# kubernetes-sigs/kube-batch

Measured on AMD Instinct MI355X. Metric: pod-node scoring evals/sec + binds/sec, 100k tasks x 10k nodes snapshot, higher is better.
Workload: dtype f64+i64

## Files before the change

### kube-batch_amd/csrc/kb_commit_sel.hip

```cpp
#include <string.h>

#include <algorithm>

#include "kb_k9.hpp"
#include "kb_repair.hpp"

#define K9S_PREP0 5u
#define K9S_PREPS 3u
#define K9S_SPIN_LIMIT (1u << 21)

__device__ __forceinline__ uint32_t k9s_ld(const uint32_t *p) { return __hip_atomic_load(p, __ATOMIC_ACQUIRE, __HIP_MEMORY_SCOPE_WORKGROUP); }
__device__ __forceinline__ void k9s_st(uint32_t *p, uint32_t v) { __hip_atomic_store(p, v, __ATOMIC_RELEASE, __HIP_MEMORY_SCOPE_WORKGROUP); }
__device__ __forceinline__ bool k9s_wait(K9Sync &Y, const uint32_t *p, uint32_t need, uint32_t nap = 1u) {
  uint32_t spins = 0;
  for (;;) {
    if (k9s_ld(p) >= need) return true;
    if ((++spins & 31u) == 0u) {
      if (k9s_ld(&Y.stop) | k9s_ld(&Y.err)) return k9s_ld(p) >= need;
      if (spins > K9S_SPIN_LIMIT) { k9s_st(&Y.err, 1u); return false; }
    }
    if (nap == 0u) { } else if (nap == 1u) __builtin_amdgcn_s_sleep(1); else if (nap <= 4u) __builtin_amdgcn_s_sleep(4); else __builtin_amdgcn_s_sleep(16);
  }
}

__global__ void __launch_bounds__(K9_THREADS) k_commit_select(const K9KernArgs ka) {
  KbCommitArgs a = ka.hot;
  {
    const unsigned char __attribute__((address_space(4))) *kp = (const unsigned char __attribute__((address_space(4))) *)__builtin_amdgcn_kernarg_segment_ptr();
    a.dev = (const KbDev *)(kp + offsetof(K9KernArgs, dev));
    a.round = (const KbRound *)(kp + offsetof(K9KernArgs, round));
  }
  extern __shared__ __align__(16) unsigned char k9_smem[];
  if ((blockIdx.x & 7u) != 0u && a.round->lists_ready != nullptr) {
    const uint32_t row = blockIdx.x - 1u - blockIdx.x / 8u;
    if (row < a.n_mrows && !KB_CHAIN_BROKEN(*a.round)) kb_repair_row<K9_THREADS>(*a.dev, *a.round, k9_smem, row, threadIdx.x);
    return;
  }
  if (k9_preamble(a)) return;
  const uint32_t tid = threadIdx.x, lane = tid & 63, wave = tid >> 6;
  const uint32_t S = a.n_mrows, W = a.n_rows;
  const K9Layout lo = k9_layout(W, S, a.L, a.NP, a.R, true);
  unsigned char *k9_base_ = k9_smem;
  K9_LDS_VIEWS(lo)
  (void)shp; (void)S; (void)dk; (void)ckey; (void)cpos;
  K9Sel &X = *reinterpret_cast<K9Sel *>(k9_smem + lo.sel);
  K9Sync &Y = X.sync;
  const unsigned long long t_start = wall_clock64();
#ifdef KB_K9_TRACE
  unsigned long long t_stage[2] = {0ull, 0ull};
  const bool staged = k9_prologue(a, lo, k9_smem, tid, 0u, t_stage);
#else
  const bool staged = k9_prologue(a, lo, k9_smem, tid, 0u);
#endif
// ... 18 lines not shown
    if (brk) atomicOr(&X.brk[tid >> 5], 1u << (tid & 31));
  }
  __syncthreads();
  if (tid < W) {
    uint32_t w = tid >> 5, mword = X.brk[w] & (0xFFFFFFFFu >> (31u - (tid & 31u)));
    while (mword == 0u) { w--; mword = X.brk[w]; }
    const uint32_t p = 32u * w + (31u - (uint32_t)__clz((int)mword));
    if ((tid - p) % K9_SEL_MAXRUN == 0u) atomicOr(&X.stm[tid >> 5], 1u << (tid & 31));
  }
  __syncthreads();
  if (tid < W && ((X.stm[tid >> 5] >> (tid & 31)) & 1u)) {
    uint32_t kidx = (uint32_t)__popc(X.stm[tid >> 5] & ((1u << (tid & 31)) - 1u));
    for (uint32_t w = 0; w < (tid >> 5); w++) kidx += (uint32_t)__popc(X.stm[w]);
    X.runs[kidx] = (uint16_t)tid;
  }
  __syncthreads();
  uint32_t K = 0;
  for (uint32_t w = 0; w < 8; w++) K += (uint32_t)__popc(X.stm[w]);
  {
    uint4 rr = make_uint4(0u, 0u, 0u, 0u);
    uint32_t i0c = 0u;
    uint32_t rlen = 0u;
    if (tid < K) { i0c = X.runs[tid]; rr = rinfo[i0c]; rlen = ((tid + 1u < K) ? (uint32_t)X.runs[tid + 1u] : W) - i0c; }
    __syncthreads();
    if (tid < K) rinfo[tid] = make_uint4(i0c | (rlen << 16), rr.y, rr.z, rr.w);
    __syncthreads();
  }

#ifdef KB_K9_TRACE
  uint32_t tacc[10] = {0, 0, 0, 0, 0, 0, 0, 0, 0, 0};
  const unsigned long long t_tab = wall_clock64();
  tacc[1] = (uint32_t)(t_stage[0] - t_start); tacc[9] = (uint32_t)(t_stage[1] - t_stage[0]); tacc[2] = (uint32_t)(t_tab - t_stage[1]);
  unsigned long long tlast = __builtin_readcyclecounter();
#define K9S_TR(k, t0) do { if (lane == 0) atomicAdd(&X.tr[k], (uint32_t)(__builtin_readcyclecounter() - (t0))); } while (0)
#define K9S_NOW() __builtin_readcyclecounter()
#else
#define K9S_TR(k, t0) do { (void)(t0); } while (0)
#define K9S_NOW() 0ull
#endif
#ifndef KB_K9_NAP_PREP
#define KB_K9_NAP_PREP 1u
#endif
  constexpr uint32_t nap_prep = KB_K9_NAP_PREP, nap_dk = 1u;
#if !defined(KB_K9_PRIO) || KB_K9_PRIO
#define K9S_SETPRIO(p) __builtin_amdgcn_s_setprio(p)
#else
#define K9S_SETPRIO(p) do { } while (0)
#endif
  const unsigned long long lt = (1ull << lane) - 1ull;
  gptrd gi, gr;
  { const KbDev &d = *a.dev; gi = (gptrd)d.idle; gr = (gptrd)d.rel; }
#define K9S_RUN_HEADER_OF(ri_)                                                                                         \
  const uint32_t hx_ = (uint32_t)__builtin_amdgcn_readfirstlane((int)(ri_).x);                                          \
  const uint32_t i0 = hx_ & 0xFFFFu, r = hx_ >> 16, s = (uint32_t)__builtin_amdgcn_readfirstlane((int)(ri_).y);          \
  const uint32_t fl0 = (uint32_t)__builtin_amdgcn_readfirstlane((int)(ri_).z), km0 = (uint32_t)__builtin_amdgcn_readfirstlane((int)(ri_).w); \
  const bool plain0 = (fl0 & 1u) && (km0 == 0u || (fl0 & 4u));                                                         \
  const bool sel_run = !a.backfill && plain0 && r >= 2u && a.whole;             \
  (void)sel_run; (void)i0;
#define K9S_RUN_SHAPE(kk)                                                                                              \
  const K9Shape sh = shapes[s];                                                                                        \
  const double *si = sinit + (size_t)s * RS;                                                                           \
  const double *rres = rowres + ((kk) % K9S_PREPS) * (uint32_t)a.R;    \
  const double *rqv = plain0 ? si : rres + 2;                                             \
  (void)rqv; (void)rres;
#define K9S_RUN_HEADER(kk)                                                                                             \
  const uint4 ri_ = rinfo[(kk)];                                                                                       \
  K9S_RUN_HEADER_OF(ri_)                                                                                               \
  K9S_RUN_SHAPE(kk)

  if (wave == 0) {
    K9S_SETPRIO(3);
    uint32_t nd = 0, n_dirty_rows = 0, n_runs = 0, n_slow = 0, i_end = 0, reason_end = KB_REASON_DONE;
    uint32_t prev_nd0 = 0, prev_pc = 0;
    bool prev_chg = true;
    bool prev_all = false;
    uint4 hd_next = rinfo[0];
    for (uint32_t k = 0; k < K; k++) {
      uint32_t lane_i = tid;
      asm volatile("" : "+v"(lane_i));
      const uint4 hd = hd_next;
      if (k + 1u < K) hd_next = rinfo[k + 1u];
      K9S_RUN_HEADER_OF(hd)
      K9_STAMP(3);
      {
        uint32_t spins = 0;
        bool ok = true;
        for (;;) {
          const uint32_t *wp = (lane_i == 0u) ? (prev_all ? &Y.seq_spec : &Y.seq_cand) : (prev_chg ? &Y.seq_dk[(lane_i - 1u) & 3u] : &Y.seq_early[(lane_i - 1u) & 3u]);
          const uint32_t v = (lane_i < 5u) ? k9s_ld(wp) : 0xFFFFFFFFu;
          if (__ballot(v < k + 1u) == 0ull) break;
          if ((++spins & 31u) == 0u && (k9s_ld(&Y.err) || spins > K9S_SPIN_LIMIT)) { k9s_st(&Y.err, 1u); ok = false; break; }
          __builtin_amdgcn_s_sleep(1);
        }
        if (!ok) { reason_end = KB_REASON_INTERNAL; i_end = i0; break; }
      }
      if (prev_all && lane_i == 0) k9s_st(&Y.seq_cand, k + 1u);
      const uint32_t ncand = Y.ncand_at[k & 3u];
      const K9Sel::Cand &CD = X.cand[k & 1u];
      const uint32_t *dk = X.dkb[k & 1u];
      uint32_t *chg = Y.chg[k & 1u];
      uint32_t ck = CD.ckey[lane_i], k1 = CD.ck1[lane_i], ckind = CD.ckind[lane_i];
      const uint32_t cpos = CD.cpos[lane_i];
      uint32_t m = (lane_i < 4u) ? (prev_chg ? Y.mdk[k & 1u][lane_i] : Y.mdko[k & 1u][lane_i]) : 0u;
      if (!prev_chg && lane_i >= 4u && lane_i - 4u < prev_pc) m = dk[prev_nd0 + lane_i - 4u];
      if (lane_i < 10u) chg[lane_i] = 0u;
      K9_STAMP(0);
      if (lane_i >= ncand) { ck = 0u; k1 = 0u; ckind = 0u; }
      m = wave_max_u32(m);
      uint32_t pc = 0, j = 0, reason = KB_REASON_DONE, n_dirty = 0, sc_dirty = 0;
      bool chg_any = false;
      bool run_done = false;
      if (!a.backfill && plain0) {
        const uint32_t cmin = (ncand == r) ? rl32(ck, r - 1u) : 0u;
        const unsigned long long deeper = __ballot(lane_i + 1u < r && ckind == 0u && k1 > cmin);
        if (ncand == r && m < cmin && !deeper) {
          const unsigned long long pipes = __ballot(lane_i < r && ckind != 0u);
          const uint32_t n_take = pipes ? (uint32_t)__ffsll((unsigned long long)pipes) : r;
          if (pipes) reason = KB_REASON_PIPELINED;
          if (lane_i < n_take) {
            const uint32_t n = nmaskbits - (ck & nmaskbits);
            ldec[i0 + lane_i] = (unsigned long long)n | ((unsigned long long)ckind << 32);
            atomicOr(&bitmap[n >> 5], 1u << (n & 31));
            if (km0) {
              const double *rqv = sinit + (size_t)s * RS;
              const uint32_t rnm = CD.crnm[lane_i];
              atomicOr(&chg[(nd + lane_i) >> 5], 1u << ((nd + lane_i) & 31));
              const bool has_map = ckind ? (rnm >> 31) : (rnm & 0x7FFFFFFFu);
              if (has_map)
                for (uint32_t mm = km0, dd = 0; mm; mm >>= 1, dd++)
                  if (mm & 1u) k9_sc_sub(ckind ? gr : gi, a.NP, dd, n, rqv[dd]);
// ... 304 lines not shown
          const uint32_t adjm1 = (!kind && has_map) ? km0 : 0u;
          uint32_t nk = 0u;
          if (more) nk = k9_eval_v(a, sh, k9_load(st), scs, gi, gr, si, adjm1, 1.0, rqv, nb, nmaskbits);
          if (km0 && has_map) {
            if (sc_lane && ((km0 >> sd) & 1u)) k9_sc_sub(kind ? gr : gi, a.NP, sd, n, rqv[sd]);
            sc_dirty = 1;
          }
          if (more) {
            if (lane_i == L) {
              if (is_new) k1 = nk;
              else if (wsel == 0) d0 = nk; else if (wsel == 1) d1 = nk; else if (wsel == 2) d2 = nk; else d3 = nk;
            }
            m = wave_max_u32(max(max(max(d0, d1), max(d2, d3)), (lane_i < pc) ? k1 : 0u));
          }
          n_dirty++;
        }
        if (kind) { j++; reason = KB_REASON_PIPELINED; break; }
      }
      }
      if (sc_dirty) __threadfence();
      const uint32_t i_next = i0 + j;
      uint32_t stop = (reason != KB_REASON_DONE || k + 1u >= K) ? 1u : 0u;
      if (!stop && a.has_aff && !a.backfill && i_next != 0u) {
        const uint32_t fln = (uint32_t)__builtin_amdgcn_readfirstlane((int)hd_next.z);
        if (fln & 2u) { reason = KB_REASON_RENORM; stop = 1u; }
      }
      if (pc) { const uint32_t cp = rl32(cpos, pc - 1u); if (lane_i == 0) cursor[s] = cp + 1u; }
      prev_nd0 = nd; prev_pc = pc; prev_all = pc == ncand;
      K9_WAVE_FENCE();
      prev_chg = chg_any;
      nd += pc; n_dirty_rows += n_dirty; n_runs += 1u; n_slow += plain0 ? 0u : 1u;
      i_end = i_next; reason_end = reason;
      if (lane_i == 0) {
        Y.nd_at[(k + 1u) & 3u] = nd;
        Y.spec_ok[(k + 1u) & 3u] = prev_all ? 1u : 0u;
        if (stop) k9s_st(&Y.stop, 1u);
        k9s_st(&Y.seq_done, k + 1u);
      }
      if (stop) break;
    }
#ifdef KB_K9_TRACE
    tacc[4] = (uint32_t)(wall_clock64() - t_tab);
#endif
    if (lane == 0) {
      if (k9s_ld(&Y.err)) reason_end = KB_REASON_INTERNAL;
      k9s_st(&Y.stop, 1u);
      H.i = i_end; H.nd = nd; H.reason = reason_end; H.n_dirty_rows = n_dirty_rows; H.n_runs = n_runs; H.n_slow = n_slow;
    }
  } else if (wave <= 4u) {
    K9S_SETPRIO(2);
    const uint32_t t = tid - 64u;
    for (uint32_t q = 0; q < K; q++) {
      K9S_RUN_HEADER(q)
      uint32_t *dko = X.dkb[q & 1u];
      uint32_t key = 0u, nd_early = 0u;
      const unsigned long long tw0 = K9S_NOW();
      if (q >= 1u) {
        if (!k9s_wait(Y, &Y.seq_done, q - 1u, nap_dk) || !k9s_wait(Y, &Y.seq_cand, q, nap_dk) || k9s_ld(&Y.stop)) break;
        nd_early = Y.nd_at[(q - 1u) & 3u] + Y.ncand_at[(q - 1u) & 3u];
        if (t < nd_early) {
          const K9St vs = k9_load(slots + (size_t)t * K9_NF);
          const K9Sc scp = k9_sc_preload(sh.active >> 2, gi, gr, a.NP, vs.node);
          key = k9_eval_v(a, sh, vs, scp, gi, gr, si, 0u, 0.0, si, nb, nmaskbits);
          dko[t] = key;
        }
        const uint32_t wmo = wave_max_u32(t < Y.nd_at[(q - 1u) & 3u] ? key : 0u);
        if (lane == 0) Y.mdko[q & 1u][wave - 1u] = wmo;
      }
      if (lane == 0) k9s_st(&Y.seq_early[wave - 1u], q + 1u);
      if (wave == 1u) K9S_TR(3, tw0);
      const unsigned long long tw1 = K9S_NOW();
      if (!k9s_wait(Y, &Y.seq_done, q, nap_dk) || k9s_ld(&Y.stop)) break;
      if (wave == 1u) K9S_TR(2, tw1);
      const uint32_t nd = Y.nd_at[q & 3u];
      if (t < nd && (t >= nd_early || ((Y.chg[(q - 1u) & 1u][t >> 5] >> (t & 31)) & 1u))) {
        const K9St vs = k9_load(slots + (size_t)t * K9_NF);
        const K9Sc scp = k9_sc_preload(sh.active >> 2, gi, gr, a.NP, vs.node);
        key = k9_eval_v(a, sh, vs, scp, gi, gr, si, 0u, 0.0, si, nb, nmaskbits);
      }
      if (t >= nd) key = 0u;
      if (t < K9_MAXSLOTS) dko[t] = key;
      const uint32_t wm = wave_max_u32(key);
      if (lane == 0) { Y.mdk[q & 1u][wave - 1u] = wm; k9s_st(&Y.seq_dk[wave - 1u], q + 1u); }
    }
  } else if (wave < K9S_PREP0 + K9S_PREPS) {
    typedef const unsigned long long __attribute__((address_space(1))) *gptr8;
    typedef const uint32_t __attribute__((address_space(1))) *gptr4;
    gptr8 g8[10];
    gptr8 gports;
    gptr4 gcls, gmaxp, gpodc, gnm;
    {
      const KbDev &d = *a.dev;
      g8[0] = (gptr8)reinterpret_cast<const unsigned long long *>(d.idle); g8[1] = (gptr8)reinterpret_cast<const unsigned long long *>(d.idle + d.NP);
      g8[2] = (gptr8)reinterpret_cast<const unsigned long long *>(d.rel); g8[3] = (gptr8)reinterpret_cast<const unsigned long long *>(d.rel + d.NP);
      g8[4] = (gptr8)reinterpret_cast<const unsigned long long *>(d.inv_acpu); g8[5] = (gptr8)reinterpret_cast<const unsigned long long *>(d.inv_amem);
      g8[6] = (gptr8)reinterpret_cast<const unsigned long long *>(d.acpu); g8[7] = (gptr8)reinterpret_cast<const unsigned long long *>(d.amem);
      g8[8] = (gptr8)reinterpret_cast<const unsigned long long *>(d.nzc); g8[9] = (gptr8)reinterpret_cast<const unsigned long long *>(d.nzm);
      gports = (gptr8)d.ports;
      gcls = (gptr4)d.ncls; gmaxp = (gptr4)reinterpret_cast<const uint32_t *>(d.maxpods); gpodc = (gptr4)reinterpret_cast<const uint32_t *>(d.podcnt); gnm = (gptr4)d.nmask;
    }
    K9Prep &P = X.prep[wave - K9S_PREP0];
    for (uint32_t m = wave - K9S_PREP0; m < K; m += K9S_PREPS) {
      K9S_RUN_HEADER(m)
      const uint32_t r1 = m >= 1u ? (uint32_t)X.runs[m] - (uint32_t)X.runs[m - 1u] : 0u, r2 = m >= 2u ? (uint32_t)X.runs[m - 1u] - (uint32_t)X.runs[m - 2u] : 0u;
      uint32_t want = r + r1 + r2, need = m >= 2u ? m - 2u : 0u;
      if (want > 64u) { want = r + r1; need = m >= 1u ? m - 1u : 0u; }
      const unsigned long long tp0 = K9S_NOW();
      if (!k9s_wait(Y, &Y.seq_done, need, nap_prep) || k9s_ld(&Y.stop)) break;
      K9S_TR(1, tp0);
      uint32_t nf = 0;
      {
        uint32_t e_ = cursor[s];
        while (nf < want) {
          const uint32_t pos_ = e_ + lane;
          const uint32_t kk_ = (pos_ < Lp) ? lists[s * Lp + pos_] : 0u;
          const bool nz_ = kk_ != 0u;
          const uint32_t nn_ = nmaskbits - (kk_ & nmaskbits);
          const bool cl_ = nz_ && !((bitmap[(nz_ ? nn_ : 0u) >> 5] >> (nn_ & 31)) & 1u);
          const unsigned long long zeros_ = __ballot(!nz_);
          const uint32_t fz_ = zeros_ ? (uint32_t)__ffsll((unsigned long long)zeros_) - 1u : 64u;
          const unsigned long long clean_ = __ballot(cl_ && lane < fz_);
          const uint32_t rank_ = (uint32_t)__popcll(clean_ & lt);
          if (((clean_ >> lane) & 1ull) && nf + rank_ < want) { P.ckey[nf + rank_] = kk_; P.cpos[nf + rank_] = pos_; }
          nf = min(want, nf + (uint32_t)__popcll(clean_));
          if (fz_ < 64u || e_ + 64u >= Lp) break;
          e_ += 64u;
        }
        K9_WAVE_FENCE();
      }
      const uint32_t key = (lane < nf) ? P.ckey[lane] : 0u, mypos = (lane < nf) ? P.cpos[lane] : 0u;
      const uint32_t n = nmaskbits - (key & nmaskbits);
      unsigned long long raw[11] = {0, 0, 0, 0, 0, 0, 0, 0, 0, 0, 0};
      uint32_t rcls = 0, rmaxp = 0, rpodc = 0, rnm = 0;
      if (lane < nf) {
#pragma unroll
        for (int f = 0; f < 10; f++) raw[f] = g8[f][n];
        raw[F_PORTS] = gports ? gports[n] : 0ull;
        rcls = gcls[n]; rmaxp = gmaxp[n]; rpodc = gpodc[n]; rnm = gnm[n];
      }
      if (!plain0 && lane == 63) {
        const KbDev &d_ = *a.dev;
        const uint32_t tk_ = desc[i0].task;
        for (int dd = 0; dd < a.R; dd++) rowres[(m % K9S_PREPS) * (uint32_t)a.R + (uint32_t)dd] = d_.t_res[(size_t)dd * d_.T + tk_];
      }
      K9_WAVE_FENCE();
      K9St v;
      uint32_t kind = 0u, k1 = 0u;
      {
        double res0 = sh.init0, res1 = sh.init1;
        if (!plain0) { res0 = rres[0]; res1 = rres[1]; }
        double idle0 = u2d(raw[F_IDLE0]), idle1 = u2d(raw[F_IDLE1]), rel0 = u2d(raw[F_REL0]), rel1 = u2d(raw[F_REL1]);
        const K9Sc scn = k9_sc_preload(sh.active >> 2, gi, gr, a.NP, lane < nf ? n : 0u);
        if (!a.backfill) {
          bool fi = le_eps(sh.init0, idle0, EPS_CPU) && le_eps(sh.init1, idle1, EPS_MEM);
          for (uint32_t aa = sh.active >> 2, dd = 0; aa; aa >>= 1, dd++)
            if (aa & 1u) fi = fi && le_eps(si[dd], k9_sci(scn, gi, a.NP, dd, lane < nf ? n : 0u), EPS_SCALAR);
          kind = fi ? 0u : 1u;
        }
        if (kind) { rel0 -= res0; rel1 -= res1; } else { idle0 -= res0; idle1 -= res1; }
        v.idle0 = idle0; v.idle1 = idle1; v.rel0 = rel0; v.rel1 = rel1;
        v.inv_ac = u2d(raw[F_INVAC]); v.inv_am = u2d(raw[F_INVAM]);
        v.ac = (double)(long long)raw[F_AC]; v.am = (double)(long long)raw[F_AM];
        v.nzc = (double)(long long)raw[F_NZC] + sh.nzc; v.nzm = (double)(long long)raw[F_NZM] + sh.nzm;
        v.ports = raw[F_PORTS] | sh.want;
        v.cls = rcls; v.node = lane < nf ? n : 0u; v.left = (int)rmaxp - (int)rpodc - 1;
        const uint32_t adjm = (!kind && (rnm & 0x7FFFFFFFu)) ? km0 : 0u;
        if (lane < nf) {
          k1 = k9_eval_v(a, sh, v, scn, gi, gr, si, adjm, 1.0, rqv, nb, nmaskbits);
        }
      }
      K9Sel::Cand &CD = X.cand[m & 1u];
      auto settle = [&](bool ahead) {
        uint32_t nd0 = Y.nd_at[m & 3u];
        bool keep = lane < nf && !((bitmap[n >> 5] >> (n & 31)) & 1u);
        if (ahead) {
          const K9Sel::Cand &CP = X.cand[(m - 1u) & 1u];
          const uint32_t ncp = Y.ncand_at[(m - 1u) & 3u];
          nd0 = Y.nd_at[(m - 1u) & 3u] + ncp;
          for (uint32_t i = 0; i < ncp; i++) keep = keep && (nmaskbits - (CP.ckey[i] & nmaskbits)) != n;
        }
        const unsigned long long kb = __ballot(keep);
        const uint32_t rho = (uint32_t)__popcll(kb & lt);
        const uint32_t ncand = min((uint32_t)__popcll(kb), r);
        if (keep && rho < r) {
          unsigned long long *st = slots + (size_t)(nd0 + rho) * K9_NF;
          st[F_IDLE0] = d2u(v.idle0); st[F_IDLE1] = d2u(v.idle1); st[F_REL0] = d2u(v.rel0); st[F_REL1] = d2u(v.rel1);
          st[F_INVAC] = raw[F_INVAC]; st[F_INVAM] = raw[F_INVAM]; st[F_AC] = d2u(v.ac); st[F_AM] = d2u(v.am);
          st[F_NZC] = d2u(v.nzc); st[F_NZM] = d2u(v.nzm); st[F_PORTS] = v.ports;
          st[F_CLS_LEFT] = (unsigned long long)rcls | ((unsigned long long)(uint32_t)v.left << 32);
          st[F_NODE_NMASK] = (unsigned long long)n | ((unsigned long long)rnm << 32);
          CD.ckey[rho] = key; CD.cpos[rho] = mypos;
          CD.ckind[rho] = kind; CD.ck1[rho] = k1; CD.crnm[rho] = rnm;
        }
        if (lane == 0) Y.ncand_at[m & 3u] = ncand;
      };
      if (m >= 1u) {
        if (!k9s_wait(Y, &Y.seq_cand, m, nap_prep) || k9s_ld(&Y.stop)) break;
        settle(true);
        if (lane == 0) k9s_st(&Y.seq_spec, m + 1u);
      }
      const unsigned long long tp1 = K9S_NOW();
      if (!k9s_wait(Y, &Y.seq_done, m, nap_prep) || k9s_ld(&Y.stop)) break;
      K9S_TR(0, tp1);
      if (m == 0u || !Y.spec_ok[m & 3u]) {
        settle(false);
        if (lane == 0) k9s_st(&Y.seq_cand, m + 1u);
      }
    }
  }
#ifdef KB_K9_TRACE
  if (tid == 0) {
    unsigned long long *tw = reinterpret_cast<unsigned long long *>(a.result);
    tw[5] = (unsigned long long)tacc[0] | ((unsigned long long)tacc[1] << 32);
    tw[6] = (unsigned long long)tacc[2] | ((unsigned long long)tacc[3] << 32);
    tw[7] = (unsigned long long)tacc[4] | ((unsigned long long)tacc[5] << 32);
    tw[13] = (unsigned long long)tacc[6] | ((unsigned long long)tacc[7] << 32);
    tw[14] = (unsigned long long)tacc[8] | ((unsigned long long)tacc[9] << 32);
  }
#endif
  __syncthreads();
#ifdef KB_K9_TRACE
  if (tid == 0) {
    unsigned long long *tw = reinterpret_cast<unsigned long long *>(a.result);
    tw[4] = (unsigned long long)X.tr[0] | ((unsigned long long)X.tr[1] << 32);
    tw[15] = (unsigned long long)X.tr[2] | ((unsigned long long)X.tr[3] << 32);
  }
#endif
  k9_epilogue(a, lo, k9_smem, tid, t_start, X.stat[0] | (X.stat[1] << 16), X.stat[2] | (X.stat[3] << 16), true, job_of_my_row);
}

void kb_launch_commit_sel(const KbDev &d, const KbRound &r, void *stream) {
  if (r.n_rows == 0) return;
  static bool lds_set[64] = {};
  k9_allow_full_lds(reinterpret_cast<const void *>(k_commit_select), lds_set);
  size_t sh = k9_layout(r.n_rows, r.n_mrows, r.L, d.NP, d.R, true).total;
  if (r.lists_ready != nullptr) sh = std::max(sh, kb_repair_lds_bytes(d.NP, K9_THREADS));
  K9KernArgs ka;
  k9_fill_args(ka, d, r);
  static_assert(KB_REPAIR_THREADS == K9_THREADS, "the repair workgroups of a fused launch are workgroups of this kernel");
// ... 7 lines not shown
```

### kube-batch_amd/csrc/kb_engine.cpp

```cpp
#include "kb_engine_int.hpp"

thread_local std::string g_create_err;

namespace kbe {

void ensure_window_buffers(kb_engine *e, uint32_t rows) {
  if (rows <= e->win_cap) return;
  if (!e->b_desc.p) e->b_desc.alloc(sizeof(KbRowDesc) * 2 * KB_K5_MAX_WINDOW);
  e->h_rows.resize(rows);
  e->h_slot.resize(rows);
  e->h_decnode.resize(rows);
  e->h_deckind.resize(rows);
  e->win_cap = rows;
}
void ensure_ip_scratch(kb_engine *e, size_t rows) {
  if (!e->hs.has_interpod) return;
  const size_t NP = e->dev.NP;
  if (e->b_ip_scnt.bytes < sizeof(long long) * rows * NP) {
    e->b_ip_scnt.alloc(sizeof(long long) * rows * NP);
    e->b_ip_shist.alloc(sizeof(int32_t) * rows * NP);
  }
  e->dev.ip_scratch_cnt = e->b_ip_scnt.as<long long>();
  e->dev.ip_scratch_hist = e->b_ip_shist.as<int32_t>();
}
// ... 148 lines not shown
  return rc;
}

void kb_engine_destroy(kb_engine *e) {
  if (!e) return;
  if (getenv("KB_K5_STATS"))
    fprintf(stderr, "[kb K5] rounds on the run kernel %llu, on the selection kernel %llu, last dirty share %.3f\n",
            (unsigned long long)e->rounds_run, (unsigned long long)e->rounds_sel, e->dirty_share);
  if (getenv("KB_K5_STATS") && e->rounds_sel)
    fprintf(stderr, "[kb select] runs of >= 2 rows: all picks clean first placements %llu, committed by shots %llu (shots cut short by a table's end %llu; shots %llu)\n",
            (unsigned long long)e->sel_stat[0], (unsigned long long)e->sel_stat[1], (unsigned long long)e->sel_stat[2], (unsigned long long)e->sel_stat[3]);
  if (getenv("KB_K5_STATS"))
    fprintf(stderr, "[kb K5] rounds %llu, rows %llu, dirty slots %llu, dirty-won rows %llu, runs %llu, runs with a row-specific Resreq %llu (%llu)\n",
            (unsigned long long)e->stats.rounds, (unsigned long long)e->stats.decisions, (unsigned long long)e->k5_slots,
            (unsigned long long)e->stats.row_fallbacks, (unsigned long long)e->k5_walks, (unsigned long long)e->k5_rescans,
            (unsigned long long)e->k5_demand);
  if (getenv("KB_K5_STATS")) fprintf(stderr, "[kb overlap] rounds with candidate lists built beside the predecessor's commit %llu, lists that never arrived %llu; repair launches: %.3f ms from their start to the tag seen\n",
                                     (unsigned long long)e->overlapped_rounds, (unsigned long long)e->overlap_faults, e->tl_repair_tag);
  if (getenv("KB_K5_STATS"))
    fprintf(stderr, "[kb host] ms over the engine's life: reset %.2f, allocate up to its first launch %.2f, speculation breaks (answer -> re-planned launch) %.2f, "
            "closing reductions %.2f, waiting for rounds %.2f, backfill up to its first launch %.2f\n", e->tl_reset, e->tl_begin, e->tl_break, e->tl_finish, e->tl_wait, e->tl_backfill);
  if (getenv("KB_K5_STATS"))
    fprintf(stderr, "[kb host] of the start: order machine %.2f, first probe %.2f, first plan %.2f; of the breaks: probe launch + absorb %.2f, waiting for the probe %.2f, re-plan %.2f\n",
            e->tl_begin_parts[0], e->tl_begin_parts[1], e->tl_begin_parts[2], e->tl_break_parts[0], e->tl_break_parts[1], e->tl_break_parts[2]);
  if (getenv("KB_K5_STATS")) fprintf(stderr, "[kb probe] %llu probes, %llu shapes marked dead by them\n", (unsigned long long)e->probes, (unsigned long long)e->probe_deaths);
  if (getenv("KB_K5_STATS") && e->k5_trace[0] > 0) {
    static const char *ph[10] = {"barrier 1 (wave 0's wait)", "evaluate: candidates (wave 0)", "barrier 2", "rows", "prepare the next run",
                                "rows, of runs with scalar dimensions", "runs with scalar dimensions (count)", "evaluate, of runs with scalar dimensions",
                                "dirty-winner entries (count)", "loop top"};
    static const char *ph_sel[10] = {"wave 0 waits for candidates + dirty keys", "staging: lists, descriptors (10 ns units, not clocks)", "run tables (10 ns units)", "rows: serial loop, tail, publish", "wave 0's loop (10 ns units)",
                                    "selection: entries + first rank", "selection: deep passes", "selection: picks + AddTask", "selection: all picks clean", "shape tables (10 ns units)"};
    const double runs = (double)(e->k5_walks ? e->k5_walks : 1);
    for (int k = 0; k < 10; k++) fprintf(stderr, "[kb K5 trace] %-32s %14.0f clocks  (%.0f per run)\n", e->rounds_sel > e->rounds_run ? ph_sel[k] : ph[k], e->k5_trace[k], e->k5_trace[k] / runs);
    static const char *ph_role[4] = {"prep waves wait for their run's turn (sum of 3)", "prep waves wait for the walk's turn (sum of 3)", "wave 1 waits for the previous run", "wave 1 evaluates + publishes"};
    if (e->rounds_sel > e->rounds_run) for (int k = 10; k < 14; k++) fprintf(stderr, "[kb K5 trace] %-32s %14.0f clocks  (%.0f per run)\n", ph_role[k - 10], e->k5_trace[k], e->k5_trace[k] / runs);
  }
  (void)hipSetDevice(e->device);
  delete e;
}

int kb_get_binds(kb_engine *e, uint32_t *task_node_out) {
  if (!e) return KB_E_INVALID;
  return guarded(e, [&]() {
    if (!e->loaded) throw EngineError(KB_E_STATE, "no session loaded");
    quiesce(e);
    HIP_OK(hipMemcpy(task_node_out, e->b_tbind.p, sizeof(uint32_t) * e->hs.T, hipMemcpyDeviceToHost));
    uint64_t nb = 0;
    for (uint32_t t = 0; t < e->hs.T; t++) nb += task_node_out[t] != KB_NONE;
    e->stats.binds = nb;
  });
}

int kb_get_task_state(kb_engine *e, uint8_t *status_out, uint32_t *node_out) {
  if (!e) return KB_E_INVALID;
  return guarded(e, [&]() {
    if (!e->loaded) throw EngineError(KB_E_STATE, "no session loaded");
    quiesce(e);
    if (status_out) HIP_OK(hipMemcpy(status_out, e->b_tstatus.p, e->hs.T, hipMemcpyDeviceToHost));
    if (node_out) HIP_OK(hipMemcpy(node_out, e->b_tnode.p, sizeof(uint32_t) * e->hs.T, hipMemcpyDeviceToHost));
  });
}

int kb_get_node_state(kb_engine *e, double *idle, double *releasing, int64_t *nz_cpu, int64_t *nz_mem, int32_t *pod_cnt) {
  if (!e) return KB_E_INVALID;
  return guarded(e, [&]() {
    if (!e->loaded) throw EngineError(KB_E_STATE, "no session loaded");
    quiesce(e);
// ... 46 lines not shown
```

### kube-batch_amd/csrc/kb_k9.hpp

```cpp
#pragma once
#include <hip/hip_runtime.h>
#include <stddef.h>
#include <stdint.h>
#include <stdlib.h>

#include "kb_device.h"
#include "kb_eval.hpp"
#include "kb_warm.hpp"

#define K9_THREADS 512
#define K9_MAXRUN 64
#define K9_SEL_MAXRUN 32
#define K9_MAXSLOTS 256
#define K9_NF 13
enum { F_IDLE0 = 0, F_IDLE1, F_REL0, F_REL1, F_INVAC, F_INVAM, F_AC, F_AM, F_NZC, F_NZM, F_PORTS, F_CLS_LEFT, F_NODE_NMASK };

struct K9Shape {
  double init0, init1, nzc, nzm;
  unsigned long long conf, want;
  uint32_t cls, active, crow, pad;
};

struct K9Hdr {
  uint32_t i, nd, reason, stop;
  uint32_t ncand, n_dirty_rows, n_runs, n_slow;
  uint32_t cur_s, cur_r, cur_fl, cur_km;
};

struct K9Prep {
  uint32_t ckey[64], cpos[64];
};
struct K9Sync {
  uint32_t seq_done;
  uint32_t seq_cand;
  uint32_t seq_dk[4];
  uint32_t seq_early[4];
  uint32_t seq_spec;
  uint32_t spec_ok[4];
  uint32_t stop, err;
  uint32_t nd_at[4];
  uint32_t ncand_at[4];
  uint32_t mdk[2][4];
  uint32_t mdko[2][4];
  uint32_t chg[2][10];
};
struct K9Sel {
  K9Sync sync;
  K9Prep prep[3];
  uint16_t runs[KB_K5_MAX_ROWS];
  uint32_t brk[8], stm[8];
  struct Cand { uint32_t ckey[64], cpos[64], ckind[64], ck1[64], crnm[64]; } cand[2];
  uint32_t dkb[2][K9_MAXSLOTS];
  uint32_t c_slot[64], c_sorted[64];
  alignas(16) uint32_t c_key[64];
  alignas(16) uint32_t e_eff[64];
  uint32_t e_key[64];
  uint32_t pool[K9_MAXSLOTS + 64];
  uint32_t tr[4];
  uint32_t stat[4];
};

struct K9Layout {
  uint32_t slots, rowres, sinit, shapes, desc, rinfo, dec, hdr, dk, ckey, cpos, cursor, shp, lists, bitmap, sel, total;
  uint32_t Lp, RS;
};
__host__ __device__ inline K9Layout k9_layout(uint32_t n_rows, uint32_t n_shapes, uint32_t L, uint32_t NP, int R, bool sel = false) {
  K9Layout o;
  o.RS = R > 2 ? (uint32_t)(R - 2) : 0u;
  o.Lp = L;
  uint32_t off = 0;
  o.slots = off;  off += (n_rows + K9_MAXRUN) * K9_NF * 8u;
  o.rowres = off; off += 3u * (uint32_t)R * 8u;
  o.sinit = off;  off += n_shapes * o.RS * 8u;
  o.shapes = off; off += n_shapes * (uint32_t)sizeof(K9Shape);
  o.desc = off;   off += n_rows * (uint32_t)sizeof(KbRowDesc);
  off = (off + 15u) & ~15u;
  o.rinfo = off;  off += n_rows * 16u;
  o.dec = off;    off += n_rows * 8u;
// ... 442 lines not shown
```

Baseline: 20.97 billion.

## Merge sync-word polls into one LDS read and skip final pass after unchanged runs

Reorders K9Sync so seq_done, seq_cand, stop and err sit in one aligned 16-byte word group, and polls all four with a single LDS vector read instead of separate atomic loads. Evaluator waves 1-4 now prefetch the next run header and shape, and skip the final re-evaluation pass when the previous run changed no slot, using a new chg_at flag published by wave 0. The aim is to cut spin-wait latency and redundant evaluation on the serial commit path. It relies on the skip being semantically safe and on the struct layout assumptions. It also shrinks spec_ok to 16-bit and adds extra trace levels.

```diff
diff --git a/kube-batch_amd/csrc/kb_commit_sel.hip b/kube-batch_amd/csrc/kb_commit_sel.hip
--- a/kube-batch_amd/csrc/kb_commit_sel.hip
+++ b/kube-batch_amd/csrc/kb_commit_sel.hip
@@ -11,14 +11,23 @@
 
 __device__ __forceinline__ uint32_t k9s_ld(const uint32_t *p) { return __hip_atomic_load(p, __ATOMIC_ACQUIRE, __HIP_MEMORY_SCOPE_WORKGROUP); }
 __device__ __forceinline__ void k9s_st(uint32_t *p, uint32_t v) { __hip_atomic_store(p, v, __ATOMIC_RELEASE, __HIP_MEMORY_SCOPE_WORKGROUP); }
-__device__ __forceinline__ bool k9s_wait(K9Sync &Y, const uint32_t *p, uint32_t need, uint32_t nap = 1u) {
+typedef uint32_t k9s_u4 __attribute__((ext_vector_type(4)));
+__device__ __forceinline__ bool k9s_wait2(K9Sync &Y, uint32_t need_done, uint32_t need_cand, uint32_t nap, uint32_t *cand = nullptr) {
+  static_assert(offsetof(K9Sync, seq_done) == 0 && offsetof(K9Sync, seq_cand) == 4 && offsetof(K9Sync, stop) == 8 && offsetof(K9Sync, err) == 12 && offsetof(K9Sel, sync) == 0 &&
+                alignof(K9Sel) >= 16, "the four words of a look are one aligned 16-byte read");
+  need_done = (uint32_t)__builtin_amdgcn_readfirstlane((int)need_done); need_cand = (uint32_t)__builtin_amdgcn_readfirstlane((int)need_cand);
   uint32_t spins = 0;
   for (;;) {
-    if (k9s_ld(p) >= need) return true;
-    if ((++spins & 31u) == 0u) {
-      if (k9s_ld(&Y.stop) | k9s_ld(&Y.err)) return k9s_ld(p) >= need;
-      if (spins > K9S_SPIN_LIMIT) { k9s_st(&Y.err, 1u); return false; }
+    const k9s_u4 v = *(const volatile k9s_u4 __attribute__((address_space(3))) *)(&Y.seq_done);
+    const uint32_t v_done = (uint32_t)__builtin_amdgcn_readfirstlane((int)v.x), v_cand = (uint32_t)__builtin_amdgcn_readfirstlane((int)v.y);
+    const uint32_t v_end = (uint32_t)__builtin_amdgcn_readfirstlane((int)(v.z | v.w));
+    if (v_done >= need_done && v_cand >= need_cand) {
+      __builtin_amdgcn_fence(__ATOMIC_ACQUIRE, "workgroup");
+      if (cand) *cand = v_cand;
+      return (uint32_t)__builtin_amdgcn_readfirstlane((int)v.z) == 0u;
     }
+    if (v_end) return false;
+    if (++spins > K9S_SPIN_LIMIT) { k9s_st(&Y.err, 1u); return false; }
     if (nap == 0u) { } else if (nap == 1u) __builtin_amdgcn_s_sleep(1); else if (nap <= 4u) __builtin_amdgcn_s_sleep(4); else __builtin_amdgcn_s_sleep(16);
   }
 }
@@ -103,9 +112,13 @@
   const unsigned long long t_tab = wall_clock64();
   tacc[1] = (uint32_t)(t_stage[0] - t_start); tacc[9] = (uint32_t)(t_stage[1] - t_stage[0]); tacc[2] = (uint32_t)(t_tab - t_stage[1]);
   unsigned long long tlast = __builtin_readcyclecounter();
-#define K9S_TR(k, t0) do { if (lane == 0) atomicAdd(&X.tr[k], (uint32_t)(__builtin_readcyclecounter() - (t0))); } while (0)
+#define K9S_TRL(lv, k, t0) do { if (KB_K9_TRACE == (lv) && lane == 0) atomicAdd(&X.tr[k], (uint32_t)(__builtin_readcyclecounter() - (t0))); } while (0)
+#define K9S_CNTL(lv, k, c) do { if (KB_K9_TRACE == (lv) && lane == 0 && (c)) atomicAdd(&X.tr[k], 1u); } while (0)
+#define K9S_TR(k, t0) K9S_TRL(1, k, t0)
 #define K9S_NOW() __builtin_readcyclecounter()
 #else
+#define K9S_TRL(lv, k, t0) do { (void)(t0); } while (0)
+#define K9S_CNTL(lv, k, c) do { } while (0)
 #define K9S_TR(k, t0) do { (void)(t0); } while (0)
 #define K9S_NOW() 0ull
 #endif
@@ -117,6 +130,9 @@
 #define K9S_SETPRIO(p) __builtin_amdgcn_s_setprio(p)
 #else
 #define K9S_SETPRIO(p) do { } while (0)
+#endif
+#ifndef KB_K9_SKIP_FINAL
+#define KB_K9_SKIP_FINAL 1
 #endif
   const unsigned long long lt = (1ull << lane) - 1ull;
   gptrd gi, gr;
@@ -128,12 +144,13 @@
   const bool plain0 = (fl0 & 1u) && (km0 == 0u || (fl0 & 4u));                                                         \
   const bool sel_run = !a.backfill && plain0 && r >= 2u && a.whole;             \
   (void)sel_run; (void)i0;
-#define K9S_RUN_SHAPE(kk)                                                                                              \
-  const K9Shape sh = shapes[s];                                                                                        \
+#define K9S_RUN_SHAPE_OF(kk, sh_)                                                                                      \
+  const K9Shape sh = (sh_);                                                                                            \
   const double *si = sinit + (size_t)s * RS;                                                                           \
   const double *rres = rowres + ((kk) % K9S_PREPS) * (uint32_t)a.R;    \
   const double *rqv = plain0 ? si : rres + 2;                                             \
   (void)rqv; (void)rres;
+#define K9S_RUN_SHAPE(kk) K9S_RUN_SHAPE_OF(kk, shapes[s])
 #define K9S_RUN_HEADER(kk)                                                                                             \
   const uint4 ri_ = rinfo[(kk)];                                                                                       \
   K9S_RUN_HEADER_OF(ri_)                                                                                               \
@@ -153,6 +170,7 @@
       if (k + 1u < K) hd_next = rinfo[k + 1u];
       K9S_RUN_HEADER_OF(hd)
       K9_STAMP(3);
+      K9S_CNTL(3, 1, k >= 1u && !prev_chg);
       {
         uint32_t spins = 0;
         bool ok = true;
@@ -539,6 +557,7 @@
       if (lane_i == 0) {
         Y.nd_at[(k + 1u) & 3u] = nd;
         Y.spec_ok[(k + 1u) & 3u] = prev_all ? 1u : 0u;
+        Y.chg_at[(k + 1u) & 3u] = chg_any ? 1u : 0u;
         if (stop) k9s_st(&Y.stop, 1u);
         k9s_st(&Y.seq_done, k + 1u);
       }
@@ -555,13 +574,25 @@
   } else if (wave <= 4u) {
     K9S_SETPRIO(2);
     const uint32_t t = tid - 64u;
+    uint4 hd_q = rinfo[0], hd_n = rinfo[K > 1u ? 1u : 0u];
+    K9Shape sh_q = shapes[(uint32_t)__builtin_amdgcn_readfirstlane((int)hd_q.y)];
+    uint32_t cand_seen = 0u;
+    bool fresh = false;
     for (uint32_t q = 0; q < K; q++) {
-      K9S_RUN_HEADER(q)
+      const unsigned long long th0 = K9S_NOW();
+      const uint4 ri_ = hd_q;
+      K9S_RUN_HEADER_OF(ri_)
+      K9S_RUN_SHAPE_OF(q, sh_q)
+      hd_q = hd_n;
+      if (q + 1u < K) sh_q = shapes[(uint32_t)__builtin_amdgcn_readfirstlane((int)hd_q.y)];
+      if (q + 2u < K) hd_n = rinfo[q + 2u];
       uint32_t *dko = X.dkb[q & 1u];
       uint32_t key = 0u, nd_early = 0u;
       const unsigned long long tw0 = K9S_NOW();
+      if (wave == 1u) { K9S_TRL(2, 0, th0); K9S_CNTL(3, 3, true); }
       if (q >= 1u) {
-        if (!k9s_wait(Y, &Y.seq_done, q - 1u, nap_dk) || !k9s_wait(Y, &Y.seq_cand, q, nap_dk) || k9s_ld(&Y.stop)) break;
+        if (!(fresh && cand_seen >= q) && !k9s_wait2(Y, q - 1u, q, nap_dk)) break;
+        if (wave == 1u) K9S_TRL(2, 1, tw0);
         nd_early = Y.nd_at[(q - 1u) & 3u] + Y.ncand_at[(q - 1u) & 3u];
         if (t < nd_early) {
           const K9St vs = k9_load(slots + (size_t)t * K9_NF);
@@ -575,10 +606,18 @@
       if (lane == 0) k9s_st(&Y.seq_early[wave - 1u], q + 1u);
       if (wave == 1u) K9S_TR(3, tw0);
       const unsigned long long tw1 = K9S_NOW();
-      if (!k9s_wait(Y, &Y.seq_done, q, nap_dk) || k9s_ld(&Y.stop)) break;
-      if (wave == 1u) K9S_TR(2, tw1);
-      const uint32_t nd = Y.nd_at[q & 3u];
-      if (t < nd && (t >= nd_early || ((Y.chg[(q - 1u) & 1u][t >> 5] >> (t & 31)) & 1u))) {
+      if (wave == 1u) K9S_TRL(2, 2, tw0);
+      fresh = false;
+      if (!k9s_wait2(Y, q, 0u, nap_dk, &cand_seen)) break;
+      if (wave == 1u) { K9S_TR(2, tw1); K9S_TRL(2, 3, tw1); }
+      const uint32_t changed = Y.chg_at[q & 3u], nd = Y.nd_at[q & 3u], chgw = Y.chg[(q - 1u) & 1u][t >> 5];
+#if KB_K9_SKIP_FINAL
+      if (q >= 1u && changed == 0u) { fresh = true; continue; }
+#else
+      (void)changed;
+#endif
+      const unsigned long long tw2 = K9S_NOW();
+      if (t < nd && (t >= nd_early || ((chgw >> (t & 31)) & 1u))) {
         const K9St vs = k9_load(slots + (size_t)t * K9_NF);
         const K9Sc scp = k9_sc_preload(sh.active >> 2, gi, gr, a.NP, vs.node);
         key = k9_eval_v(a, sh, vs, scp, gi, gr, si, 0u, 0.0, si, nb, nmaskbits);
@@ -587,6 +626,7 @@
       if (t < K9_MAXSLOTS) dko[t] = key;
       const uint32_t wm = wave_max_u32(key);
       if (lane == 0) { Y.mdk[q & 1u][wave - 1u] = wm; k9s_st(&Y.seq_dk[wave - 1u], q + 1u); }
+      if (wave == 1u) { K9S_TRL(3, 0, tw2); K9S_CNTL(3, 2, true); }
     }
   } else if (wave < K9S_PREP0 + K9S_PREPS) {
     typedef const unsigned long long __attribute__((address_space(1))) *gptr8;
@@ -611,7 +651,7 @@
       uint32_t want = r + r1 + r2, need = m >= 2u ? m - 2u : 0u;
       if (want > 64u) { want = r + r1; need = m >= 1u ? m - 1u : 0u; }
       const unsigned long long tp0 = K9S_NOW();
-      if (!k9s_wait(Y, &Y.seq_done, need, nap_prep) || k9s_ld(&Y.stop)) break;
+      if (!k9s_wait2(Y, need, 0u, nap_prep)) break;
       K9S_TR(1, tp0);
       uint32_t nf = 0;
       {
@@ -700,12 +740,12 @@
         if (lane == 0) Y.ncand_at[m & 3u] = ncand;
       };
       if (m >= 1u) {
-        if (!k9s_wait(Y, &Y.seq_cand, m, nap_prep) || k9s_ld(&Y.stop)) break;
+        if (!k9s_wait2(Y, 0u, m, nap_prep)) break;
         settle(true);
         if (lane == 0) k9s_st(&Y.seq_spec, m + 1u);
       }
       const unsigned long long tp1 = K9S_NOW();
-      if (!k9s_wait(Y, &Y.seq_done, m, nap_prep) || k9s_ld(&Y.stop)) break;
+      if (!k9s_wait2(Y, m, 0u, nap_prep)) break;
       K9S_TR(0, tp1);
       if (m == 0u || !Y.spec_ok[m & 3u]) {
         settle(false);
diff --git a/kube-batch_amd/csrc/kb_engine.cpp b/kube-batch_amd/csrc/kb_engine.cpp
--- a/kube-batch_amd/csrc/kb_engine.cpp
+++ b/kube-batch_amd/csrc/kb_engine.cpp
@@ -204,7 +204,13 @@
                                     "selection: entries + first rank", "selection: deep passes", "selection: picks + AddTask", "selection: all picks clean", "shape tables (10 ns units)"};
     const double runs = (double)(e->k5_walks ? e->k5_walks : 1);
     for (int k = 0; k < 10; k++) fprintf(stderr, "[kb K5 trace] %-32s %14.0f clocks  (%.0f per run)\n", e->rounds_sel > e->rounds_run ? ph_sel[k] : ph[k], e->k5_trace[k], e->k5_trace[k] / runs);
+#if defined(KB_K9_TRACE) && KB_K9_TRACE == 2
+    static const char *ph_role[4] = {"wave 1: run header + shape", "wave 1 waits for run q - 2 and run q - 1's candidates", "wave 1: that wait + early evaluation + publish", "wave 1 waits for run q - 1 (seq_done >= q)"};
+#elif defined(KB_K9_TRACE) && KB_K9_TRACE == 3
+    static const char *ph_role[4] = {"wave 1: final pass", "runs behind a run that changed no slot (count)", "final passes made by wave 1 (count)", "runs wave 1 saw (count)"};
+#else
     static const char *ph_role[4] = {"prep waves wait for their run's turn (sum of 3)", "prep waves wait for the walk's turn (sum of 3)", "wave 1 waits for the previous run", "wave 1 evaluates + publishes"};
+#endif
     if (e->rounds_sel > e->rounds_run) for (int k = 10; k < 14; k++) fprintf(stderr, "[kb K5 trace] %-32s %14.0f clocks  (%.0f per run)\n", ph_role[k - 10], e->k5_trace[k], e->k5_trace[k] / runs);
   }
   (void)hipSetDevice(e->device);
diff --git a/kube-batch_amd/csrc/kb_k9.hpp b/kube-batch_amd/csrc/kb_k9.hpp
--- a/kube-batch_amd/csrc/kb_k9.hpp
+++ b/kube-batch_amd/csrc/kb_k9.hpp
@@ -33,11 +33,12 @@
 struct K9Sync {
   uint32_t seq_done;
   uint32_t seq_cand;
+  uint32_t stop, err;
   uint32_t seq_dk[4];
   uint32_t seq_early[4];
   uint32_t seq_spec;
-  uint32_t spec_ok[4];
-  uint32_t stop, err;
+  uint16_t spec_ok[4];
+  uint16_t chg_at[4];
   uint32_t nd_at[4];
   uint32_t ncand_at[4];
   uint32_t mdk[2][4];
```

New measurement: 21.32 billion, median of 6. No clear change (+1.7%).

## Pack sync payloads into 64-bit sequence words for the commit-select waves

Applied to the files above, without the earlier changes.

Replaces the separate sequence counters and side arrays (nd_at, ncand_at, spec_ok) with 64-bit atomic words that carry the sequence number together with a payload holding nd, ncand and the spec/chg/stop flags. Waiters get the state in the same acquire load that releases them, so they skip extra LDS reads and separate stop checks. The dk waves also skip the full recompute when the previous round had no changes, prefetch the next shape header, and pin kernel arguments in scalar registers. The cost is tighter bitfield limits (slots under 512) and more intricate ordering logic that could break under races.

```diff
diff --git a/kube-batch_amd/csrc/kb_commit_sel.hip b/kube-batch_amd/csrc/kb_commit_sel.hip
--- a/kube-batch_amd/csrc/kb_commit_sel.hip
+++ b/kube-batch_amd/csrc/kb_commit_sel.hip
@@ -11,13 +11,22 @@
 
 __device__ __forceinline__ uint32_t k9s_ld(const uint32_t *p) { return __hip_atomic_load(p, __ATOMIC_ACQUIRE, __HIP_MEMORY_SCOPE_WORKGROUP); }
 __device__ __forceinline__ void k9s_st(uint32_t *p, uint32_t v) { __hip_atomic_store(p, v, __ATOMIC_RELEASE, __HIP_MEMORY_SCOPE_WORKGROUP); }
-__device__ __forceinline__ bool k9s_wait(K9Sync &Y, const uint32_t *p, uint32_t need, uint32_t nap = 1u) {
+__device__ __forceinline__ unsigned long long k9s_ld64(const unsigned long long *p) { return __hip_atomic_load(p, __ATOMIC_ACQUIRE, __HIP_MEMORY_SCOPE_WORKGROUP); }
+__device__ __forceinline__ void k9s_st64(unsigned long long *p, uint32_t seq, uint32_t payload) {
+  __hip_atomic_store(p, (unsigned long long)seq | ((unsigned long long)payload << 32), __ATOMIC_RELEASE, __HIP_MEMORY_SCOPE_WORKGROUP);
+}
+__device__ __forceinline__ bool k9s_wait(K9Sync &Y, const unsigned long long *p, uint32_t need, uint32_t nap, uint32_t &seq, uint32_t &pay) {
   uint32_t spins = 0;
   for (;;) {
-    if (k9s_ld(p) >= need) return true;
-    if ((++spins & 31u) == 0u) {
-      if (k9s_ld(&Y.stop) | k9s_ld(&Y.err)) return k9s_ld(p) >= need;
-      if (spins > K9S_SPIN_LIMIT) { k9s_st(&Y.err, 1u); return false; }
+    unsigned long long w = k9s_ld64(p);
+    bool ok = (uint32_t)w >= need, out = ok;
+    if (!ok && (++spins & 31u) == 0u) {
+      if (k9s_ld(&Y.stop) | k9s_ld(&Y.err)) { w = k9s_ld64(p); ok = (uint32_t)w >= need; out = true; }
+      else if (spins > K9S_SPIN_LIMIT) { k9s_st(&Y.err, 1u); out = true; }
+    }
+    if (out) {
+      seq = (uint32_t)__builtin_amdgcn_readfirstlane((int)(uint32_t)w); pay = (uint32_t)__builtin_amdgcn_readfirstlane((int)(uint32_t)(w >> 32));
+      return ok;
     }
     if (nap == 0u) { } else if (nap == 1u) __builtin_amdgcn_s_sleep(1); else if (nap <= 4u) __builtin_amdgcn_s_sleep(4); else __builtin_amdgcn_s_sleep(16);
   }
@@ -145,6 +154,7 @@
     uint32_t prev_nd0 = 0, prev_pc = 0;
     bool prev_chg = true;
     bool prev_all = false;
+    uint32_t prev_cf = 0;
     uint4 hd_next = rinfo[0];
     for (uint32_t k = 0; k < K; k++) {
       uint32_t lane_i = tid;
@@ -153,20 +163,24 @@
       if (k + 1u < K) hd_next = rinfo[k + 1u];
       K9S_RUN_HEADER_OF(hd)
       K9_STAMP(3);
+      unsigned long long pw;
       {
         uint32_t spins = 0;
         bool ok = true;
         for (;;) {
-          const uint32_t *wp = (lane_i == 0u) ? (prev_all ? &Y.seq_spec : &Y.seq_cand) : (prev_chg ? &Y.seq_dk[(lane_i - 1u) & 3u] : &Y.seq_early[(lane_i - 1u) & 3u]);
-          const uint32_t v = (lane_i < 5u) ? k9s_ld(wp) : 0xFFFFFFFFu;
-          if (__ballot(v < k + 1u) == 0ull) break;
+          const unsigned long long *wp = (lane_i == 0u) ? (prev_all ? &Y.seq_spec : &Y.seq_cand) : (prev_chg ? &Y.seq_dk[(lane_i - 1u) & 3u] : &Y.seq_early[(lane_i - 1u) & 3u]);
+          pw = (lane_i < 5u) ? k9s_ld64(wp) : ~0ull;
+          if (__ballot((uint32_t)pw < k + 1u) == 0ull) break;
           if ((++spins & 31u) == 0u && (k9s_ld(&Y.err) || spins > K9S_SPIN_LIMIT)) { k9s_st(&Y.err, 1u); ok = false; break; }
           __builtin_amdgcn_s_sleep(1);
         }
         if (!ok) { reason_end = KB_REASON_INTERNAL; i_end = i0; break; }
       }
-      if (prev_all && lane_i == 0) k9s_st(&Y.seq_cand, k + 1u);
-      const uint32_t ncand = Y.ncand_at[k & 3u];
+      const uint32_t cf = (uint32_t)(pw >> 32) & 0x7FFFu;
+      if ((uint32_t)__builtin_amdgcn_readfirstlane((int)(uint32_t)pw) != k + 1u) { k9s_st(&Y.err, 1u); reason_end = KB_REASON_INTERNAL; i_end = i0; break; }
+      if (prev_all && lane_i == 0) k9s_st64(&Y.seq_cand, k + 1u, cf | (prev_cf << 15));
+      prev_cf = cf;
+      const uint32_t ncand = (uint32_t)__builtin_amdgcn_readfirstlane((int)cf) >> 9;
       const K9Sel::Cand &CD = X.cand[k & 1u];
       const uint32_t *dk = X.dkb[k & 1u];
       uint32_t *chg = Y.chg[k & 1u];
@@ -537,10 +551,8 @@
       nd += pc; n_dirty_rows += n_dirty; n_runs += 1u; n_slow += plain0 ? 0u : 1u;
       i_end = i_next; reason_end = reason;
       if (lane_i == 0) {
-        Y.nd_at[(k + 1u) & 3u] = nd;
-        Y.spec_ok[(k + 1u) & 3u] = prev_all ? 1u : 0u;
         if (stop) k9s_st(&Y.stop, 1u);
-        k9s_st(&Y.seq_done, k + 1u);
+        k9s_st64(&Y.seq_done, k + 1u, nd | (prev_nd0 << 9) | (prev_all ? K9S_DONE_SPEC : 0u) | (chg_any ? K9S_DONE_CHG : 0u) | (stop ? K9S_DONE_STOP : 0u));
       }
       if (stop) break;
     }
@@ -555,38 +567,59 @@
   } else if (wave <= 4u) {
     K9S_SETPRIO(2);
     const uint32_t t = tid - 64u;
+    KbCommitArgs ae = a;
+    KbDev de;
+    de.compat = a.dev->compat; de.n_nc = a.dev->n_nc;
+    asm volatile("" : "+s"(ae.fit_mode), "+s"(ae.pred_enabled), "+s"(ae.score_enabled), "+s"(ae.use_crow), "+s"(ae.NP), "+s"(ae.wL), "+s"(ae.wM), "+s"(ae.wB), "+s"(de.compat), "+s"(de.n_nc));
+    ae.dev = &de;
+    uint4 hd_next = rinfo[0];
+    K9Shape sh_next = shapes[(uint32_t)__builtin_amdgcn_readfirstlane((int)hd_next.y)];
     for (uint32_t q = 0; q < K; q++) {
-      K9S_RUN_HEADER(q)
+      const uint4 hd = hd_next;
+      const K9Shape sh = sh_next;
+      hd_next = rinfo[min(q + 1u, K - 1u)];
+      K9S_RUN_HEADER_OF(hd)
+      (void)r; (void)plain0;
+      const double *si = sinit + (size_t)s * RS;
       uint32_t *dko = X.dkb[q & 1u];
       uint32_t key = 0u, nd_early = 0u;
+      uint32_t sq, py;
       const unsigned long long tw0 = K9S_NOW();
       if (q >= 1u) {
-        if (!k9s_wait(Y, &Y.seq_done, q - 1u, nap_dk) || !k9s_wait(Y, &Y.seq_cand, q, nap_dk) || k9s_ld(&Y.stop)) break;
-        nd_early = Y.nd_at[(q - 1u) & 3u] + Y.ncand_at[(q - 1u) & 3u];
+        if (!k9s_wait(Y, &Y.seq_cand, q, nap_dk, sq, py)) break;
+        if (sq > q + 1u) { if (lane == 0) k9s_st(&Y.err, 1u); break; }
+        const uint32_t cfp = (sq == q ? py : py >> 15) & 0x7FFFu;
+        nd_early = cfp & 511u;
         if (t < nd_early) {
           const K9St vs = k9_load(slots + (size_t)t * K9_NF);
-          const K9Sc scp = k9_sc_preload(sh.active >> 2, gi, gr, a.NP, vs.node);
-          key = k9_eval_v(a, sh, vs, scp, gi, gr, si, 0u, 0.0, si, nb, nmaskbits);
+          const K9Sc scp = k9_sc_preload(sh.active >> 2, gi, gr, ae.NP, vs.node);
+          key = k9_eval_v(ae, sh, vs, scp, gi, gr, si, 0u, 0.0, si, nb, nmaskbits);
           dko[t] = key;
         }
-        const uint32_t wmo = wave_max_u32(t < Y.nd_at[(q - 1u) & 3u] ? key : 0u);
+        const uint32_t wmo = wave_max_u32(t < nd_early - (cfp >> 9) ? key : 0u);
         if (lane == 0) Y.mdko[q & 1u][wave - 1u] = wmo;
       }
-      if (lane == 0) k9s_st(&Y.seq_early[wave - 1u], q + 1u);
+      if (lane == 0) k9s_st64(&Y.seq_early[wave - 1u], q + 1u, 0u);
+      sh_next = shapes[(uint32_t)__builtin_amdgcn_readfirstlane((int)hd_next.y)];
       if (wave == 1u) K9S_TR(3, tw0);
       const unsigned long long tw1 = K9S_NOW();
-      if (!k9s_wait(Y, &Y.seq_done, q, nap_dk) || k9s_ld(&Y.stop)) break;
+      if (!k9s_wait(Y, &Y.seq_done, q, nap_dk, sq, py)) break;
       if (wave == 1u) K9S_TR(2, tw1);
-      const uint32_t nd = Y.nd_at[q & 3u];
-      if (t < nd && (t >= nd_early || ((Y.chg[(q - 1u) & 1u][t >> 5] >> (t & 31)) & 1u))) {
-        const K9St vs = k9_load(slots + (size_t)t * K9_NF);
-        const K9Sc scp = k9_sc_preload(sh.active >> 2, gi, gr, a.NP, vs.node);
-        key = k9_eval_v(a, sh, vs, scp, gi, gr, si, 0u, 0.0, si, nb, nmaskbits);
-      }
+      if (sq > q + 1u) { if (lane == 0) k9s_st(&Y.err, 1u); break; }
+      if (py & K9S_DONE_STOP) break;
+      const uint32_t nd = (sq == q ? py : py >> 9) & 511u;
       if (t >= nd) key = 0u;
+      if (q == 0u || (sq == q && (py & K9S_DONE_CHG))) {
+        if (t < nd && (t >= nd_early || ((Y.chg[(q - 1u) & 1u][t >> 5] >> (t & 31)) & 1u))) {
+          const K9St vs = k9_load(slots + (size_t)t * K9_NF);
+          const K9Sc scp = k9_sc_preload(sh.active >> 2, gi, gr, ae.NP, vs.node);
+          key = k9_eval_v(ae, sh, vs, scp, gi, gr, si, 0u, 0.0, si, nb, nmaskbits);
+        }
+        const uint32_t wm = wave_max_u32(key);
+        if (lane == 0) Y.mdk[q & 1u][wave - 1u] = wm;
+      }
       if (t < K9_MAXSLOTS) dko[t] = key;
-      const uint32_t wm = wave_max_u32(key);
-      if (lane == 0) { Y.mdk[q & 1u][wave - 1u] = wm; k9s_st(&Y.seq_dk[wave - 1u], q + 1u); }
+      if (lane == 0) k9s_st64(&Y.seq_dk[wave - 1u], q + 1u, 0u);
     }
   } else if (wave < K9S_PREP0 + K9S_PREPS) {
     typedef const unsigned long long __attribute__((address_space(1))) *gptr8;
@@ -611,7 +644,8 @@
       uint32_t want = r + r1 + r2, need = m >= 2u ? m - 2u : 0u;
       if (want > 64u) { want = r + r1; need = m >= 1u ? m - 1u : 0u; }
       const unsigned long long tp0 = K9S_NOW();
-      if (!k9s_wait(Y, &Y.seq_done, need, nap_prep) || k9s_ld(&Y.stop)) break;
+      uint32_t sq, py;
+      if (!k9s_wait(Y, &Y.seq_done, need, nap_prep, sq, py) || (py & K9S_DONE_STOP)) break;
       K9S_TR(1, tp0);
       uint32_t nf = 0;
       {
@@ -675,13 +709,10 @@
         }
       }
       K9Sel::Cand &CD = X.cand[m & 1u];
-      auto settle = [&](bool ahead) {
-        uint32_t nd0 = Y.nd_at[m & 3u];
+      auto settle = [&](bool ahead, const uint32_t nd0, const uint32_t ncp) -> uint32_t {
         bool keep = lane < nf && !((bitmap[n >> 5] >> (n & 31)) & 1u);
         if (ahead) {
           const K9Sel::Cand &CP = X.cand[(m - 1u) & 1u];
-          const uint32_t ncp = Y.ncand_at[(m - 1u) & 3u];
-          nd0 = Y.nd_at[(m - 1u) & 3u] + ncp;
           for (uint32_t i = 0; i < ncp; i++) keep = keep && (nmaskbits - (CP.ckey[i] & nmaskbits)) != n;
         }
         const unsigned long long kb = __ballot(keep);
@@ -697,19 +728,22 @@
           CD.ckey[rho] = key; CD.cpos[rho] = mypos;
           CD.ckind[rho] = kind; CD.ck1[rho] = k1; CD.crnm[rho] = rnm;
         }
-        if (lane == 0) Y.ncand_at[m & 3u] = ncand;
+        return K9S_CAND(nd0 + ncand, ncand);
       };
+      uint32_t cfp = 0u;
       if (m >= 1u) {
-        if (!k9s_wait(Y, &Y.seq_cand, m, nap_prep) || k9s_ld(&Y.stop)) break;
-        settle(true);
-        if (lane == 0) k9s_st(&Y.seq_spec, m + 1u);
+        if (!k9s_wait(Y, &Y.seq_cand, m, nap_prep, sq, py)) break;
+        if (sq != m) { if (lane == 0) k9s_st(&Y.err, 1u); break; }
+        cfp = py & 0x7FFFu;
+        const uint32_t cfa = settle(true, cfp & 511u, cfp >> 9);
+        if (lane == 0) k9s_st64(&Y.seq_spec, m + 1u, cfa);
       }
       const unsigned long long tp1 = K9S_NOW();
-      if (!k9s_wait(Y, &Y.seq_done, m, nap_prep) || k9s_ld(&Y.stop)) break;
+      if (!k9s_wait(Y, &Y.seq_done, m, nap_prep, sq, py) || (py & K9S_DONE_STOP)) break;
       K9S_TR(0, tp1);
-      if (m == 0u || !Y.spec_ok[m & 3u]) {
-        settle(false);
-        if (lane == 0) k9s_st(&Y.seq_cand, m + 1u);
+      if (sq == m && (m == 0u || !(py & K9S_DONE_SPEC))) {
+        const uint32_t cfb = settle(false, py & 511u, 0u);
+        if (lane == 0) k9s_st64(&Y.seq_cand, m + 1u, cfb | (cfp << 15));
       }
     }
   }
diff --git a/kube-batch_amd/csrc/kb_k9.hpp b/kube-batch_amd/csrc/kb_k9.hpp
--- a/kube-batch_amd/csrc/kb_k9.hpp
+++ b/kube-batch_amd/csrc/kb_k9.hpp
@@ -30,20 +30,22 @@
 struct K9Prep {
   uint32_t ckey[64], cpos[64];
 };
+#define K9S_DONE_SPEC (1u << 18)
+#define K9S_DONE_CHG (1u << 19)
+#define K9S_DONE_STOP (1u << 20)
+#define K9S_CAND(end, ncand) ((end) | ((ncand) << 9))
 struct K9Sync {
-  uint32_t seq_done;
-  uint32_t seq_cand;
-  uint32_t seq_dk[4];
-  uint32_t seq_early[4];
-  uint32_t seq_spec;
-  uint32_t spec_ok[4];
+  unsigned long long seq_done;
+  unsigned long long seq_cand;
+  unsigned long long seq_spec;
+  unsigned long long seq_dk[4];
+  unsigned long long seq_early[4];
   uint32_t stop, err;
-  uint32_t nd_at[4];
-  uint32_t ncand_at[4];
   uint32_t mdk[2][4];
   uint32_t mdko[2][4];
   uint32_t chg[2][10];
 };
+static_assert(K9_MAXSLOTS + K9_SEL_MAXRUN < 512 && K9_SEL_MAXRUN < 64, "K9S_CAND's fields");
 struct K9Sel {
   K9Sync sync;
   K9Prep prep[3];
```

Result: slower. 21.13 billion before, 20.87 billion after (-1.3%).
